# Vi-Sri/CerebralSignalNetworks

Hardware: AMD Instinct MI355X
Metric: EEG-segments/sec training (128ch x 500, hidden=768) (higher is better)
Workload: dtype bf16

## Files before the change

### cerebralsignalnetworks_amd/csrc/csn_common.h

```cpp
#pragma once
#include <hip/hip_runtime.h>
#include <stdint.h>
#include <stdio.h>
#include <stdlib.h>
#include <atomic>
#include <string>

#include "../../include/csn_hip.h"

namespace csn {

typedef __bf16 bf16_t;
typedef __attribute__((ext_vector_type(8))) __bf16 bf16x8;
typedef __attribute__((ext_vector_type(4))) __bf16 bf16x4;
typedef __attribute__((ext_vector_type(4))) float f32x4;
typedef __attribute__((ext_vector_type(4))) short s16x4;

void set_error(const std::string& msg);
int fail(int status, const char* fmt, ...);

#define CSN_HIP_CHECK(expr)                                                              \
  do {                                                                                   \
    hipError_t _e = (expr);                                                              \
    if (_e != hipSuccess)                                                                \
      return ::csn::fail(CSN_ERR_HIP, "%s failed: %s (%s:%d)", #expr, hipGetErrorString(_e), \
                         __FILE__, __LINE__);                                            \
  } while (0)

#define CSN_LAUNCH_CHECK()                                                               \
  do {                                                                                   \
    hipError_t _e = hipGetLastError();                                                   \
    if (_e != hipSuccess)                                                                \
      return ::csn::fail(CSN_ERR_HIP, "kernel launch failed: %s (%s:%d)",                \
                         hipGetErrorString(_e), __FILE__, __LINE__);                     \
  } while (0)

#define CSN_REQUIRE(cond, ...)                                                           \
  do {                                                                                   \
    if (!(cond)) return ::csn::fail(CSN_ERR_INVALID_ARGUMENT, __VA_ARGS__);              \
  } while (0)

struct Options {
  bool cell_v1, no_persist, no_persist_bwd, persist_streams, no_xcd_local, no_rotate, no_fuse_x, no_beside,
      no_side_stream, fwd_ksplit, fwd_nsplit, fwd_flags, bwd_flags, dpoll_no_hint, fwd_hint, gemm_no_dma, gemm_no_256, gemm_generic, tn_no_tr, tn_no_stagger, filter_v1, tags_no_rearm, gemm_no_192, no_half_tiles, nt_no_w4, no_fwd_park;
  int chunk;
  int tn_stages;
};
static inline Options options_from_env() {
  auto on = [](const char* name) { return getenv(name) != nullptr; };
  auto num = [](const char* name, int dflt) {
    const char* e = getenv(name);
    return e ? atoi(e) : dflt;
  };
  Options o{};
  o.cell_v1 = on("CSN_CELL_V1");
  o.no_persist = on("CSN_NO_PERSIST");
  o.no_persist_bwd = on("CSN_NO_PERSIST_BWD");
  o.persist_streams = on("CSN_PERSIST_STREAMS");
  o.no_xcd_local = on("CSN_NO_XCD_LOCAL");
  o.no_rotate = on("CSN_NO_ROTATE");
  o.no_fuse_x = on("CSN_NO_FUSE_X");
  o.no_beside = on("CSN_NO_BESIDE");
  o.no_half_tiles = on("CSN_NO_HALF_TILES");
  o.no_fwd_park = on("CSN_NO_FWD_PARK");
  o.no_side_stream = on("CSN_NO_SIDE_STREAM");
  o.fwd_ksplit = on("CSN_FWD_KSPLIT");
  o.fwd_nsplit = on("CSN_FWD_NSPLIT");
  o.fwd_flags = on("CSN_FWD_FLAGS");
  o.bwd_flags = on("CSN_BWD_FLAGS");
  o.dpoll_no_hint = on("CSN_DPOLL_NO_HINT");
  o.fwd_hint = on("CSN_FWD_HINT");
  o.tn_no_stagger = on("CSN_TN_NO_STAGGER");
  o.gemm_no_dma = on("CSN_GEMM_NO_DMA");
  o.gemm_no_256 = on("CSN_GEMM_NO_256");
  o.gemm_no_192 = on("CSN_GEMM_NO_192");
  o.nt_no_w4 = on("CSN_NT_NO_W4");
  o.gemm_generic = on("CSN_GEMM_GENERIC");
  o.tn_no_tr = on("CSN_TN_NO_TR");
  o.filter_v1 = on("CSN_FILTER_V1");
#ifdef CSN_SLAB_TAGS
  o.tags_no_rearm = on("CSN_TAGS_NO_REARM");
#endif
  o.chunk = num("CSN_LSTM_CHUNK", 32);
  if (o.chunk < 1) o.chunk = 1;
  o.tn_stages = num("CSN_TN_STAGES", 4);
  return o;
}

static inline hipStream_t as_stream(csnStream_t s) { return reinterpret_cast<hipStream_t>(s); }
template <auto Kernel>
static int ensure_dyn_lds(int bytes) {
  static std::atomic<unsigned> done{0u};
  int dev = 0;
  CSN_HIP_CHECK(hipGetDevice(&dev));
  const unsigned bit = 1u << (dev & 31);
  if ((done.load(std::memory_order_acquire) & bit) == 0u) {
    CSN_HIP_CHECK(hipFuncSetAttribute(reinterpret_cast<const void*>(Kernel), hipFuncAttributeMaxDynamicSharedMemorySize, bytes));
    done.fetch_or(bit, std::memory_order_release);
  }
  return CSN_OK;
}

static inline size_t align_up(size_t v, size_t a) { return (v + a - 1) / a * a; }
static inline size_t dtype_size(int dtype) { return dtype == CSN_BF16 ? 2 : 4; }

__device__ __forceinline__ float to_f32(float v) { return v; }
__device__ __forceinline__ float to_f32(bf16_t v) { return (float)v; }
template <typename T> __device__ __forceinline__ T from_f32(float v);
template <> __device__ __forceinline__ float from_f32<float>(float v) { return v; }
template <> __device__ __forceinline__ bf16_t from_f32<bf16_t>(float v) { return (bf16_t)v; }

__device__ __forceinline__ float sigmoid_f32(float x) { return 1.0f / (1.0f + expf(-x)); }
__device__ __forceinline__ float tanh_f32(float x) { return tanhf(x); }

struct CellFwdOne {
// ... 45 lines not shown
```

### cerebralsignalnetworks_amd/csrc/gemm_beside.h

```cpp
#pragma once
#include "gemm_tile.h"
#include "lstm_cell_blk.h"

namespace csn {

static constexpr int kBesideStages = 3;
static constexpr unsigned kBesideStageBytes = 49152;
static constexpr unsigned kBesideLdsBytes = kBesideStages * kBesideStageBytes;

__device__ __forceinline__ void beside_gemm_tiles(const BesideGemm& g, char* smem, unsigned worker, unsigned nworkers) {
  constexpr int NSTAGE = kBesideStages;
  const int tid = threadIdx.x, lane = tid & 63, wave = tid >> 6;
  const int wm = wave >> 1, wn = wave & 1;
  const int64_t M = g.M, N = g.N, K = g.K;
  const unsigned ntn = (unsigned)((N + 127) / 128);
  const unsigned ntiles = ntn * (unsigned)((M + 255) / 256);
  const int nk = (int)(K / 64);
  const unsigned sw = (unsigned)((lane & 15) >> 1);
  const unsigned a_base = (unsigned)((wm * 128 + (lane & 15)) * 128) + ((((unsigned)lane >> 4) ^ sw) << 4);
  const unsigned b_base = 32768u + (unsigned)((wn * 64 + (lane & 15)) * 128) + ((((unsigned)lane >> 4) ^ sw) << 4);

  for (unsigned lid = worker; lid < ntiles; lid += nworkers) {
    __syncthreads();
    const int64_t m0 = (int64_t)(lid / ntn) * 256, n0 = (int64_t)(lid % ntn) * 128;
    const int srow = lane >> 3;
    auto issue = [&](int kt) {
      char* a_s = smem + (kt % NSTAGE) * kBesideStageBytes;
      char* b_s = a_s + 32768;
#pragma unroll
      for (int i = 0; i < 8; ++i) {
        const int row = (4 * i + wave) * 8 + srow;
        const int ch = (lane & 7) ^ ((row >> 1) & 7);
        int64_t am = m0 + row;
        am = am < M ? am : M - 1;
        glds16(g.A + am * K + (int64_t)kt * 64 + ch * 8, a_s + (4 * i + wave) * 1024);
      }
#pragma unroll
      for (int i = 0; i < 4; ++i) {
        const int row = (4 * i + wave) * 8 + srow;
        const int ch = (lane & 7) ^ ((row >> 1) & 7);
        int64_t bn = n0 + row;
        bn = bn < N ? bn : N - 1;
        glds16(g.Bt + bn * K + (int64_t)kt * 64 + ch * 8, b_s + (4 * i + wave) * 1024);
      }
    };

    f32x4 acc[8][4];
#pragma unroll
    for (int i = 0; i < 8; ++i)
#pragma unroll
      for (int j = 0; j < 4; ++j) acc[i][j] = (f32x4){0.f, 0.f, 0.f, 0.f};

#pragma unroll
    for (int h = 0; h < NSTAGE - 1; ++h)
      if (h < nk) issue(h);
    for (int kt = 0; kt < nk; ++kt) {
      const int ahead = nk - 1 - kt;
      if (ahead >= NSTAGE - 2) asm volatile("s_waitcnt vmcnt(%0)" ::"n"(12 * (NSTAGE - 2)) : "memory");
      else asm volatile("s_waitcnt vmcnt(0)" ::: "memory");
      __builtin_amdgcn_s_barrier();
      if (kt + NSTAGE - 1 < nk) issue(kt + NSTAGE - 1);
      const unsigned sb = (unsigned)(kt % NSTAGE) * kBesideStageBytes;
#pragma unroll
      for (int kk = 0; kk < 2; ++kk) {
        const unsigned xo = kk ? 64u : 0u;
        bf16x8 af[8], bfr[4];
#pragma unroll
        for (int j = 0; j < 4; ++j) bfr[j] = lds_read_b128(((b_base ^ xo) + sb) + j * 2048u);
#pragma unroll
        for (int i = 0; i < 8; ++i) af[i] = lds_read_b128(((a_base ^ xo) + sb) + i * 2048u);
#pragma unroll
        for (int i = 0; i < 8; ++i) {
          switch (7 - i) {
            case 7: asm volatile("s_waitcnt lgkmcnt(7)" ::: "memory"); break;
            case 6: asm volatile("s_waitcnt lgkmcnt(6)" ::: "memory"); break;
            case 5: asm volatile("s_waitcnt lgkmcnt(5)" ::: "memory"); break;
            case 4: asm volatile("s_waitcnt lgkmcnt(4)" ::: "memory"); break;
            case 3: asm volatile("s_waitcnt lgkmcnt(3)" ::: "memory"); break;
            case 2: asm volatile("s_waitcnt lgkmcnt(2)" ::: "memory"); break;
            case 1: asm volatile("s_waitcnt lgkmcnt(1)" ::: "memory"); break;
            default: asm volatile("s_waitcnt lgkmcnt(0)" ::: "memory"); break;
          }
          __builtin_amdgcn_sched_barrier(0);
#pragma unroll
          for (int j = 0; j < 4; ++j)
            acc[i][j] = __builtin_amdgcn_mfma_f32_16x16x32_bf16(bfr[j], af[i], acc[i][j], 0, 0, 0);
          __builtin_amdgcn_sched_barrier(0);
        }
      }
    }

#pragma unroll
    for (int i = 0; i < 8; ++i) {
      const int64_t m = m0 + wm * 128 + i * 16 + (lane & 15);
      if (m >= M) continue;
#pragma unroll
      for (int j = 0; j < 4; ++j) {
        const int64_t n = n0 + wn * 64 + j * 16 + (lane >> 4) * 4;
        if (n + 3 < N) {
          *reinterpret_cast<float4*>(g.C + m * N + n) = make_float4(acc[i][j][0], acc[i][j][1], acc[i][j][2], acc[i][j][3]);
        } else {
          for (int r = 0; r < 4; ++r)
            if (n + r < N) g.C[m * N + n + r] = acc[i][j][r];
        }
      }
    }
  }
  asm volatile("s_waitcnt vmcnt(0)" ::: "memory");
}

}
```

### cerebralsignalnetworks_amd/csrc/gemm_nt.hip

```cpp
#include "gemm_tile.h"

namespace csn {

template <typename OutT>
__global__ void __launch_bounds__(256)
gemm_nt_bf16_kernel(const bf16_t* __restrict__ A, const bf16_t* __restrict__ Bt, const float* __restrict__ bias,
                    OutT* __restrict__ C, int64_t M, int64_t N, int64_t K, int accumulate) {
  extern __shared__ __attribute__((aligned(16))) char smem[];
  const int tid = threadIdx.x, lane = tid & 63, wave = tid >> 6;
  const int wm = wave >> 1, wn = wave & 1;
  const unsigned ntn = (unsigned)((N + 127) / 128);
  const unsigned lid = xcd_remap(blockIdx.x, gridDim.x);
  const int64_t m0 = (int64_t)(lid / ntn) * 128, n0 = (int64_t)(lid % ntn) * 128;
  const int nk = (int)((K + 63) / 64);

  uint4 ra[4], rb[4];
  auto load_tile = [&](int kt) {
#pragma unroll
    for (int i = 0; i < 4; ++i) {
      const int q = tid + i * 256;
      const int row = q >> 3, ch = q & 7;
      const int64_t k = (int64_t)kt * 64 + ch * 8;
      const int64_t am = m0 + row, bn = n0 + row;
      ra[i] = (am < M && k < K) ? *reinterpret_cast<const uint4*>(A + am * K + k) : make_uint4(0, 0, 0, 0);
// ... 318 lines not shown
  issue_a(0);
  issue_b(0);
  if (nk > 1) issue_a(1);
  for (int kt = 0; kt < nk; ++kt) {
    if (kt + 1 < nk) asm volatile("s_waitcnt vmcnt(4)" ::: "memory");
    else asm volatile("s_waitcnt vmcnt(0)" ::: "memory");
    __builtin_amdgcn_s_barrier();
    if (kt + 1 < nk) issue_b(kt + 1);
    if (kt + 2 < nk) issue_a(kt + 2);
    const unsigned sa = (unsigned)(kt % 3) * 32768u, sb = (unsigned)(kt % 2) * kBStage;
#pragma unroll
    for (int kk = 0; kk < 2; ++kk) {
      const unsigned xo = kk ? 64u : 0u;
      bf16x8 af[4], bfr[NBF];
#pragma unroll
      for (int j = 0; j < NBF; ++j) bfr[j] = lds_read_b128(((b_base ^ xo) + sb) + j * 2048u);
#pragma unroll
      for (int i = 0; i < 4; ++i) af[i] = lds_read_b128(((a_base ^ xo) + sa) + i * 2048u);
#pragma unroll
      for (int i = 0; i < 4; ++i) {
        if (i == 0) asm volatile("s_waitcnt lgkmcnt(3)" ::: "memory");
        else if (i == 1) asm volatile("s_waitcnt lgkmcnt(2)" ::: "memory");
        else if (i == 2) asm volatile("s_waitcnt lgkmcnt(1)" ::: "memory");
        else asm volatile("s_waitcnt lgkmcnt(0)" ::: "memory");
        __builtin_amdgcn_sched_barrier(0);
#pragma unroll
        for (int j = 0; j < NBF; ++j)
          acc[i][j] = __builtin_amdgcn_mfma_f32_16x16x32_bf16(bfr[j], af[i], acc[i][j], 0, 0, 0);
        __builtin_amdgcn_sched_barrier(0);
      }
    }
  }

#pragma unroll
  for (int i = 0; i < 4; ++i) {
    const int64_t m = m0 + wm * 64 + i * 16 + (lane & 15);
    if (m >= M) continue;
#pragma unroll
    for (int j = 0; j < NBF; ++j) {
      const int64_t n = n0 + wn * (BN / 2) + j * 16 + (lane >> 4) * 4;
      const f32x4 v = nt_with_bias(acc[i][j], bias, n);
#if defined(CSN_NT_ABL) && CSN_NT_ABL == 1
      if (v[0] == v[0]) continue;
#endif
      nt_store4<OutT>(v, C, m * N + n, accumulate);
    }
  }
  }
}

#ifndef CSN_NT_W4_NA
#define CSN_NT_W4_NA 3
#endif
__device__ __forceinline__ int nt64_sw(int row) {
  const int g = (row >> 2) & 3;
  return (((g ^ (g >> 1)) & 1) << 1) | (g >> 1);
}
template <typename OutT, int NA>
__global__ void __launch_bounds__(256, 2)
gemm_nt_w4_kernel(const bf16_t* __restrict__ A, const bf16_t* __restrict__ Bt, const float* __restrict__ bias,
                  OutT* __restrict__ C, int64_t M, int64_t N, int64_t K, int accumulate) {
  static_assert(NA == 2 || NA == 3, "A ring depth");
  constexpr unsigned kAStage = 16384u, kBStage = 12288u, kBBase = NA * kAStage;
  static_assert(kBBase + 2 * kBStage <= 81920u, "two workgroups per CU");
  extern __shared__ __attribute__((aligned(1024))) char smem[];
  const int tid = threadIdx.x, lane = tid & 63;
  const int wave = __builtin_amdgcn_readfirstlane(tid >> 6);
  const int wm = wave >> 1, wn = wave & 1;
  const unsigned ntn = (unsigned)(N / 192);
  const unsigned lid = xcd_remap(blockIdx.x, gridDim.x);
  const int64_t m0 = (int64_t)(lid / ntn) * 256, n0 = (int64_t)(lid % ntn) * 192;
  const int nk = __builtin_amdgcn_readfirstlane((int)(K / 32));

  unsigned a_off[4], b_off[3];
#pragma unroll
  for (int i = 0; i < 4; ++i) {
    const int row = (4 * i + wave) * 16 + (lane >> 2);
    const int ch = (lane & 3) ^ nt64_sw(row);
    int64_t am = m0 + row;
    am = am < M ? am : M - 1;
    a_off[i] = (unsigned)((am * K + ch * 8) * 2);
  }
#pragma unroll
  for (int i = 0; i < 3; ++i) {
    const int row = (4 * i + wave) * 16 + (lane >> 2);
    const int ch = (lane & 3) ^ nt64_sw(row);
    b_off[i] = (unsigned)(((n0 + row) * K + ch * 8) * 2);
  }
  auto issue_a = [&](int kt, int i) {
    glds16(reinterpret_cast<const char*>(A + (int64_t)kt * 32) + a_off[i], smem + (unsigned)(kt % NA) * kAStage + (4 * i + wave) * 1024);
  };
  auto issue_b = [&](int kt, int i) {
    glds16(reinterpret_cast<const char*>(Bt + (int64_t)kt * 32) + b_off[i], smem + kBBase + (unsigned)(kt & 1) * kBStage + (4 * i + wave) * 1024);
  };

  const unsigned frag = (unsigned)((lane & 15) * 64) + ((((unsigned)lane >> 4) ^ (unsigned)nt64_sw(lane & 15)) << 4);
  const unsigned a_base = (unsigned)(wm * 128 * 64) + frag;
  const unsigned b_base = kBBase + (unsigned)(wn * 96 * 64) + frag;
#define W4_READ(addr, off) ({ bf16x8 v_; asm volatile("ds_read_b128 %0, %1 offset:%2" : "=v"(v_) : "v"(addr), "n"(off) : "memory"); v_; })

  f32x4 acc[8][6];
#pragma unroll
  for (int i = 0; i < 8; ++i)
#pragma unroll
    for (int j = 0; j < 6; ++j) acc[i][j] = (f32x4){0.f, 0.f, 0.f, 0.f};

#pragma unroll
  for (int i = 0; i < 4; ++i) issue_a(0, i);
#pragma unroll
  for (int i = 0; i < 3; ++i) issue_b(0, i);
// ... 128 lines not shown
```

### cerebralsignalnetworks_amd/csrc/gemm_tile.h

```cpp
#pragma once
#include "csn_common.h"

namespace csn {

__device__ __forceinline__ unsigned xcd_remap(unsigned bid, unsigned nwg) {
  const unsigned q = nwg >> 3, r = nwg & 7, xcd = bid & 7, slot = bid >> 3;
  return (xcd < r ? xcd * (q + 1) : r * (q + 1) + (xcd - r) * q) + slot;
}

__device__ __forceinline__ int nt_lds_off(int row, int chunk) {
  return row * 128 + ((chunk ^ ((row >> 1) & 7)) << 4);
}

__device__ __forceinline__ int tn_lds_off(int krow, int col) {
  const int s = (krow & 3) | (((krow >> 3) & 1) << 2);
  return krow * 256 + ((((col >> 4) ^ s) << 4) + (col & 15)) * 2;
}
__device__ __forceinline__ int tn256_lds_off(int krow, int col) {
  const int sw = (krow & 3) | (((krow >> 3) & 1) << 2);
  return krow * 512 + ((((col >> 4) ^ sw) << 4) + (col & 15)) * 2;
}

typedef __attribute__((address_space(3))) void* lds_ptr_t;
typedef const __attribute__((address_space(1))) void* gbl_ptr_t;

__device__ __forceinline__ void glds16(const void* g, void* l) {
  __builtin_amdgcn_global_load_lds((gbl_ptr_t)g, (lds_ptr_t)l, 16, 0, 0);
}

template <bool CLAMP>
__device__ __forceinline__ const bf16_t* nt_dma_src(const bf16_t* P, int64_t r0, int64_t rows, int64_t K, int piece, int lane) {
  const int row = piece * 8 + (lane >> 3);
  const int ch = (lane & 7) ^ ((row >> 1) & 7);
  int64_t r = r0 + row;
  if (CLAMP) r = r < rows ? r : rows - 1;
  return P + r * K + ch * 8;
}

__device__ __forceinline__ bf16x8 lds_read_b128(unsigned addr) {
  bf16x8 v;
  asm volatile("ds_read_b128 %0, %1" : "=v"(v) : "v"(addr) : "memory");
  return v;
}

template <typename OutT>
__device__ __forceinline__ void nt_store4(f32x4 v, OutT* __restrict__ C, int64_t idx, int accumulate) {
  if constexpr (sizeof(OutT) == 4) {
    f32x4* dst = reinterpret_cast<f32x4*>((float*)C + idx);
    if (accumulate) v += *dst;
    *dst = v;
  } else {
    *reinterpret_cast<bf16x4*>((bf16_t*)C + idx) = (bf16x4){(bf16_t)v[0], (bf16_t)v[1], (bf16_t)v[2], (bf16_t)v[3]};
  }
}
template <typename OutT>
__device__ __forceinline__ void nt_store1(float v, OutT* __restrict__ C, int64_t idx, int accumulate) {
  if constexpr (sizeof(OutT) == 4) {
    float* dst = (float*)C + idx;
    *dst = accumulate ? *dst + v : v;
  } else {
    ((bf16_t*)C)[idx] = (bf16_t)v;
  }
}
__device__ __forceinline__ f32x4 nt_with_bias(f32x4 v, const float* __restrict__ bias, int64_t n) {
// ... 33 lines not shown
```

### cerebralsignalnetworks_amd/csrc/lstm.hip

```cpp
#include <algorithm>
#include <cstring>
#include <vector>

#include "csn_common.h"
#include "lstm_cell_blk.h"
#include "lstm_cell_common.h"
#include "lstm_dropout.h"
#include "lstm_f32_persist.h"
#include "lstm_resident.h"

namespace csn {

struct LayerWs {
  size_t wih, whh, whht, wiht, whh_blk, whht_blk, bias, xproj, gates, c_all, h_all, dgates, dx, dc_carry, hblk[2],
      dgblk[2], h_blk_all, counters, dg_blk_all, bflags;
  size_t h_drop;
};
struct WsLayout {
  LayerWs layer[8];
  size_t x_c, x_blk, wih0_blk, dy_tm, tn_scratch, colsum, status, agree, agree_b, zeros_bh, f32_bias_part, total;
  size_t zero_fwd, zero_fwd_bytes, zero_bwd, zero_bwd_bytes;
  bool fuse_x;
  bool il, persist, persist_bwd;
  bool fwd_ns;
// ... 1579 lines not shown
      const int cr = r / Cz;
      const bool last = (r == T - 1);
      if (l > 0 || last) {
        if ((rc = hand_off(sc, st, side))) return rc;
      }
      if (l > 0) {
        if ((rc = dx_chunk_gemm(C, l, cr, A.dh_n, side))) return rc;
        hipEvent_t ev;
        if ((rc = next_event(sc, &ev))) return rc;
        CSN_HIP_CHECK(hipEventRecord(ev, side));
        dx_ready[(size_t)l * nch + cr] = ev;
      } else if (last && A.dx != nullptr) {
        if ((rc = dx_out(C, A.dx, side))) return rc;
      }
      if (last && (rc = weight_grads_blk(C, A, l, side))) return rc;
    }
  }
  if ((rc = prof_end(C, 1, n_launch, n_cells))) return rc;
  if ((rc = hand_off(sc, side, st))) return rc;
  for (int l = NL - 1; l >= 0; --l) C.P.grads_ready(l);
  return CSN_OK;
}

static int backward_persist(Call& C, const BwdArgs& A) {
  Plan& P = C.P;
  const WsLayout& w = C.w;
  Prof& g_prof = P.prof;
  char* ws = C.ws;
  hipStream_t st = C.st;
  const float* dh_n = A.dh_n;
  const int B = C.B, T = C.T, H = C.H, NL = C.NL;
  const int64_t G = C.G;
  const int Bpad = (B + 63) / 64 * 64, MT = Bpad / 64;
  const int Cz = C.Cz;
  const int nch = (T + Cz - 1) / Cz;
  const bool beside = NL > 1 && NL <= 4 && bwd_persist_slices(H) <= 28 && G % 64 == 0 && !P.opt.no_beside;
  const int lag = beside ? 2 : 1;
  const int ndiag = nch + lag * (NL - 1);
  int rc;
  CSN_HIP_CHECK(hipMemsetAsync(ws + w.zero_bwd, 0, w.zero_bwd_bytes, st));
  for (int l = 0; l < NL; ++l)
    if ((rc = seed_dc_carry(C, l, A.dc_n, true))) return rc;
  struct DhAdd { int l, t_lo, t_hi; };
  auto add_dh_n = [&](const DhAdd& q) -> int {
    return add_dh_n_rows(C, dh_n + (size_t)(q.l - 1) * B * H, (float*)(ws + w.layer[q.l].dx), q.t_lo, q.t_hi, st);
  };
  const bool try_local = !P.opt.no_xcd_local;

  PersistBwdArgs a{};
  a.error_flag = (unsigned*)(ws + w.status);
  a.B = B; a.H = H; a.T = T; a.Bpad = Bpad; a.MT = MT;
  a.xcd_groups = 1;
  a.grid_slices = 32;
  a.rotate = !P.opt.no_rotate;
  a.data_polls = P.opt.bwd_flags ? 0 : (P.opt.dpoll_no_hint ? 2 : 1);
#ifdef CSN_SLAB_TAGS
  if (a.data_polls && P.opt.tags_no_rearm) a.data_polls |= 4;
#endif
  P.dgates_copies = 2;
  if (a.data_polls)
    for (int l = 0; l < NL; ++l) CSN_HIP_CHECK(hipMemsetAsync(ws + w.layer[l].dg_blk_all, 0xff, (size_t)4 * Bpad * G * 2, st));
  int n_launch = 0;
  P.half_launches[1] = 0;
  BesideGemm pending[3];
  DhAdd pending_add[3] = {{0, 0, 0}, {0, 0, 0}, {0, 0, 0}};
  DhAdd pending_drop[3] = {{0, 0, 0}, {0, 0, 0}, {0, 0, 0}};
  int npending = 0;
  if ((rc = prof_mark(g_prof, 2, st))) return rc;
  for (int dg = 0; dg < ndiag; ++dg) {
    int lay[4], chk[4], ns = 0;
    for (int l = NL - 1; l >= 0; --l) {
      const int c = dg - lag * (NL - 1 - l);
      if (c < 0 || c >= nch) continue;
      const LayerWs& L = w.layer[l];
      PersistBwdSlot& S = a.slot[ns];
      S.wt_blk = (const bf16_t*)(ws + L.whht_blk);
      S.gates = (const bf16_t*)(ws + L.gates);
      S.c_all = (const float*)(ws + L.c_all);
      if (l == NL - 1) {
        S.dy = A.dy_tm;
        S.dy_last = A.dy_tm ? nullptr : A.dy_last;
      } else {
        S.dy = (const float*)(ws + w.layer[l + 1].dx);
        S.dy_last = nullptr;
      }
      S.zeros = (const float*)(ws + w.zeros_bh);
      S.dc_carry = (float*)(ws + L.dc_carry);
      S.dgates = (bf16_t*)(ws + L.dgates);
      S.dg_blk_all = (bf16_t*)(ws + L.dg_blk_all);
      S.flags = (unsigned*)(ws + L.bflags);
      const Chunk k = chunk_at(C, c);
      S.t_hi = T - 1 - k.t0;
      S.nsteps = k.nsteps;
      lay[ns] = l;
      chk[ns] = c;
      ++ns;
    }
    if (ns == 0) {
      for (int i = 0; i < npending; ++i) {
        const BesideGemm& g = pending[i];
        if ((rc = gemm_nt(g.A, g.Bt, nullptr, g.C, g.M, g.N, g.K, CSN_BF16, CSN_F32, 0, st, P.opt))) return rc;
        if ((rc = drop_bwd(C, pending_drop[i].l - 1, pending_drop[i].t_lo, pending_drop[i].t_hi, st))) return rc;
        if (pending_add[i].l && (rc = add_dh_n(pending_add[i]))) return rc;
      }
      npending = 0;
      continue;
// ... 307 lines not shown
```

### cerebralsignalnetworks_amd/csrc/lstm_bwd_persist.hip

```cpp
#include "csn_common.h"
#include "lstm_cell_common.h"
#include "lstm_cell_blk.h"
#include "gemm_beside.h"

#ifdef CSN_PSTAMPS
#ifndef CSN_STAMP_BLOCK
#define CSN_STAMP_BLOCK 11
#endif
__device__ unsigned long long g_bstamps[16];
#define CSN_BSTAMP(i)                                                          \
  do {                                                                         \
    __builtin_amdgcn_sched_barrier(0);                                         \
    if (tid == 0 && blockIdx.x == CSN_STAMP_BLOCK) {                           \
      const unsigned long long now_ = wall_clock64();                          \
      atomicAdd(&g_bstamps[i], now_ - last_);                                  \
      last_ = now_;                                                            \
    }                                                                          \
    __builtin_amdgcn_sched_barrier(0);                                         \
  } while (0)
#else
#define CSN_BSTAMP(i)
#endif

namespace csn {
// ... 4 lines not shown

static constexpr int kBwdRedTile = 68;
__device__ __forceinline__ int bwd_red_pos(int r, int q) { return (r >> 1) + 8 * (r & 1) + 17 * q; }

typedef __attribute__((ext_vector_type(4))) unsigned bu32x4;

__device__ __forceinline__ bf16x8 bload_sc1_b128(__amdgpu_buffer_rsrc_t rsrc, unsigned byte_off, int soff = 0) {
  bu32x4 v = __builtin_amdgcn_raw_buffer_load_b128(rsrc, (int)byte_off, soff, 16);
  union { bu32x4 u; bf16x8 b; } cvt;
  cvt.u = v;
  return cvt.b;
}
template <bool WT>
__device__ __forceinline__ void bstore_b128(__amdgpu_buffer_rsrc_t rsrc, unsigned byte_off, const bf16x8& v, int soff = 0) {
  union { bu32x4 u; bf16x8 b; } cvt;
  cvt.b = v;
  __builtin_amdgcn_raw_buffer_store_b128(cvt.u, rsrc, (int)byte_off, soff, WT ? 16 : 0);
}

struct PersistLens { const int* lengths; };
struct PersistNoLens {};
template <bool MASK> struct PersistLensArg { typedef PersistNoLens type; };
template <> struct PersistLensArg<true> { typedef PersistLens type; };

template <int NUT, int KS, bool DPOLL, bool MASK = false, int RG = 4>
__global__ void __launch_bounds__(256) lstm_bwd_persist_kernel(PersistBwdArgs a, typename PersistLensArg<MASK>::type lens) {
#ifndef CSN_BWD_RING
#define CSN_BWD_RING 5
#endif
  constexpr int RING = KS >= 32 ? 3 : (KS < CSN_BWD_RING ? KS : CSN_BWD_RING);
  static_assert(RG == 4 || RG == 2, "tiles of 64 or 32 rows");
  constexpr int NT = RG * NUT;
  constexpr int QPR = 4 * NUT;
  constexpr int NPAIR = 16 * RG * QPR;
  constexpr int NPASS = NPAIR / 256;
  static_assert(NPAIR % 256 == 0, "tile must split evenly over the 256 threads");
  extern __shared__ __attribute__((aligned(16))) float4 red[];
  const int B = a.B, H = a.H, MT = a.MT, T = a.T;
  const int tid = threadIdx.x, lane = tid & 63, wave = tid >> 6;
#ifdef CSN_PSTAMPS
  const unsigned long long t_entry_ = wall_clock64();
#endif
  const int nslices = H / (16 * NUT);
  int grp, slice;
  if (a.xcd_groups) {
    grp = blockIdx.x & 7;
    slice = blockIdx.x >> 3;
    const int ngroups = a.nslots * MT, gs = a.grid_slices;
    if (grp >= ngroups || slice >= nslices) {
      if (a.ngemm > 0) {
        const int idle_here = gs - nslices;
        const unsigned base = grp <= ngroups ? (unsigned)(grp * idle_here)
                                             : (unsigned)(ngroups * idle_here + (grp - ngroups) * gs);
        const unsigned worker = base + (unsigned)(grp < ngroups ? slice - nslices : slice);
        const unsigned nworkers = (unsigned)(ngroups * idle_here + (8 - ngroups) * gs);
        for (int i = 0; i < a.ngemm; ++i) beside_gemm_tiles(a.gemm[i], reinterpret_cast<char*>(red), worker, nworkers);
      }
      return;
    }
  } else {
    grp = blockIdx.x / nslices;
    slice = blockIdx.x % nslices;
  }
  const PersistBwdSlot& S = a.slot[grp / MT];
  const int mt = grp % MT;
  const int u0 = slice * 16 * NUT, m0 = mt * 16 * RG;
  const int K = 4 * H, kblocks = K >> 5;
  const int ks_beg = wave * KS;
  const size_t slab = (size_t)a.Bpad * K;
  const bf16_t* const wt_blk = S.wt_blk;
  const bf16_t* const gates = S.gates;
  const float* const c_all = S.c_all;
  const float* const dy = S.dy;
  const float* const dy_last = S.dy_last;
  bf16_t* const dgates = S.dgates;
  bf16_t* const dg_blk_all = S.dg_blk_all;
  unsigned* const flags = S.flags + (size_t)mt * kPersistFlagLine;
  const size_t flag_step = (size_t)MT * kPersistFlagLine;
  const int t_hi = S.t_hi, nsteps = S.nsteps;
  constexpr bool dpoll = DPOLL;

  bool local = false;
  if (a.xcd_groups && a.agree != nullptr) {
    if (tid == 0) {
      const unsigned xcc = __builtin_amdgcn_s_getreg(6164) & 7u;
      const unsigned long long mine = 1ull | (1ull << (8 + 6 * xcc));
      __hip_atomic_fetch_add(a.agree + grp, mine, __ATOMIC_RELAXED, __HIP_MEMORY_SCOPE_AGENT);
      const unsigned long long t_begin = wall_clock64();
      unsigned long long v;
      while (((v = __hip_atomic_load(a.agree + grp, __ATOMIC_RELAXED, __HIP_MEMORY_SCOPE_AGENT)) & 0xffull) <
             (unsigned long long)nslices) {
        __builtin_amdgcn_s_sleep(1);
        if (__hip_atomic_load(a.error_flag, __ATOMIC_RELAXED, __HIP_MEMORY_SCOPE_AGENT) != 0u) break;
        if (wall_clock64() - t_begin > kBwdSpinTimeoutTicks) {
          __hip_atomic_store(a.error_flag, 1u, __ATOMIC_RELAXED, __HIP_MEMORY_SCOPE_AGENT);
          break;
        }
      }
      ((__attribute__((address_space(3))) int*)(__attribute__((address_space(3))) void*)red)[0] = (int)(((v >> (8 + 6 * xcc)) & 63ull) == (unsigned long long)nslices);
    }
    __syncthreads();
    local = ((__attribute__((address_space(3))) int*)(__attribute__((address_space(3))) void*)red)[0] != 0;
    __syncthreads();
  }

  const int rot = a.rotate ? (slice * KS) / nslices : 0;
  bf16x8 wreg[KS][NUT];
#pragma unroll
  for (int kb = 0; kb < KS; ++kb) {
// ... 323 lines not shown
        bstore_b128<false>(slabs_rsrc, o1, hi, dst_off);
      } else {
        bstore_b128<true>(slabs_rsrc, o0, lo, dst_off);
        bstore_b128<true>(slabs_rsrc, o1, hi, dst_off);
      }
      bf16x8* op = reinterpret_cast<bf16x8*>(dgates + ((size_t)t * B + row) * K + 4 * (size_t)uq);
      nt_store(op, lo);
      nt_store(op + 1, hi);
      dcn[ps] = make_float4(dcarry[0], dcarry[1], dcarry[2], dcarry[3]);
      cc[ps] = cpv[ps];
    }
    CSN_BSTAMP(3);
    if (!dpoll) asm volatile("s_waitcnt vmcnt(0)" ::: "memory");
    __syncthreads();
    CSN_BSTAMP(4);
    if (!dpoll && tid == 0) {
      unsigned* fl = flags + (size_t)t * flag_step + slice;
      if (local) *fl = 1u;
      else __hip_atomic_store(fl, 1u, __ATOMIC_RELAXED, __HIP_MEMORY_SCOPE_AGENT);
    }
    CSN_BSTAMP(5);
  }

#pragma unroll
  for (int ps = 0; ps < NPASS; ++ps)
    if (pok[ps]) *reinterpret_cast<float4*>(S.dc_carry + (size_t)prow[ps] * H + puq[ps]) = dcn[ps];
}

bool bwd_persist_supported(int B, int H, int dtype, const Options& opt) {
  if (dtype != CSN_BF16 || opt.no_persist || opt.no_persist_bwd) return false;
  return H == 128 || H == 256 || H == 384 || H == 512 || H == 768 || H == 1024;
}
int bwd_persist_slices(int H) { return H / 32; }

template <int NUT, int KS>
static int launch_bwd_persist_t(const PersistBwdArgs& a, hipStream_t st, const int* lengths) {
  size_t lds = (size_t)4 * (a.half_tiles ? 2 : 4) * NUT * kBwdRedTile * sizeof(float4);
  if (lengths != nullptr) {
    if (int rc = ensure_dyn_lds<&lstm_bwd_persist_kernel<NUT, KS, false, true>>((int)kBesideLdsBytes)) return rc;
    if (int rc = ensure_dyn_lds<&lstm_bwd_persist_kernel<NUT, KS, true, true>>((int)kBesideLdsBytes)) return rc;
  } else if (a.half_tiles) {
    if (int rc = ensure_dyn_lds<&lstm_bwd_persist_kernel<NUT, KS, false, false, 2>>((int)kBesideLdsBytes)) return rc;
    if (int rc = ensure_dyn_lds<&lstm_bwd_persist_kernel<NUT, KS, true, false, 2>>((int)kBesideLdsBytes)) return rc;
  } else {
    if (int rc = ensure_dyn_lds<&lstm_bwd_persist_kernel<NUT, KS, false>>((int)kBesideLdsBytes)) return rc;
    if (int rc = ensure_dyn_lds<&lstm_bwd_persist_kernel<NUT, KS, true>>((int)kBesideLdsBytes)) return rc;
  }
  const unsigned nslices = (unsigned)(a.H / (16 * NUT));
  PersistBwdArgs b = a;
  if (b.xcd_groups) {
    if (b.ngemm > 0) {
      lds = kBesideLdsBytes;
      if (b.grid_slices < (int)nslices) b.grid_slices = (int)nslices;
    } else {
      b.grid_slices = (int)nslices;
    }
  }
  const unsigned grid = b.xcd_groups ? 8u * (unsigned)b.grid_slices : nslices * (unsigned)(b.MT * b.nslots);
  if (lengths != nullptr) {
    const PersistLens pl{lengths};
    if (b.data_polls) lstm_bwd_persist_kernel<NUT, KS, true, true><<<dim3(grid), 256, lds, st>>>(b, pl);
    else lstm_bwd_persist_kernel<NUT, KS, false, true><<<dim3(grid), 256, lds, st>>>(b, pl);
  } else if (b.half_tiles) {
    if (b.data_polls) lstm_bwd_persist_kernel<NUT, KS, true, false, 2><<<dim3(grid), 256, lds, st>>>(b, PersistNoLens{});
    else lstm_bwd_persist_kernel<NUT, KS, false, false, 2><<<dim3(grid), 256, lds, st>>>(b, PersistNoLens{});
  } else if (b.data_polls) lstm_bwd_persist_kernel<NUT, KS, true><<<dim3(grid), 256, lds, st>>>(b, PersistNoLens{});
  else lstm_bwd_persist_kernel<NUT, KS, false><<<dim3(grid), 256, lds, st>>>(b, PersistNoLens{});
  CSN_LAUNCH_CHECK();
  return CSN_OK;
}

int launch_bwd_persist(const PersistBwdArgs& a, hipStream_t st, const int* lengths) {
  CSN_REQUIRE(a.nslots >= 1 && a.nslots <= 4 && a.MT >= 1, "launch_bwd_persist: bad slot count");
  const int ns = bwd_persist_slices(a.H);
  CSN_REQUIRE(ns % 4 == 0 && ns <= kPersistFlagLine, "launch_bwd_persist: H=%d gives %d slices", a.H, ns);
  if (a.xcd_groups) CSN_REQUIRE(a.nslots * a.MT <= 8, "launch_bwd_persist: groups do not fit 8 XCDs");
  CSN_REQUIRE(a.MT * (a.half_tiles ? 32 : 64) == a.Bpad, "launch_bwd_persist: %d tiles of %d rows are not Bpad=%d", a.MT,
              a.half_tiles ? 32 : 64, a.Bpad);
  CSN_REQUIRE(!a.half_tiles || (a.xcd_groups && lengths == nullptr), "launch_bwd_persist: 32-row groups need the grouped form and no lengths");
  CSN_REQUIRE(a.ngemm >= 0 && a.ngemm <= 3 && (a.ngemm == 0 || a.xcd_groups), "launch_bwd_persist: bad GEMM list");
  for (int i = 0; i < a.ngemm; ++i)
    CSN_REQUIRE(a.gemm[i].K % 64 == 0 && a.gemm[i].N % 4 == 0 && a.gemm[i].M > 0, "launch_bwd_persist: GEMM %d shape", i);
  switch (a.H) {
    case 1024: return launch_bwd_persist_t<2, 32>(a, st, lengths);
    case 768: return launch_bwd_persist_t<2, 24>(a, st, lengths);
    case 512: return launch_bwd_persist_t<2, 16>(a, st, lengths);
    case 384: return launch_bwd_persist_t<2, 12>(a, st, lengths);
    case 256: return launch_bwd_persist_t<2, 8>(a, st, lengths);
    case 128: return launch_bwd_persist_t<2, 4>(a, st, lengths);
  }
  return fail(CSN_ERR_UNSUPPORTED, "launch_bwd_persist: no kernel for H=%d", a.H);
}

}

#ifdef CSN_PSTAMPS
extern "C" int csn_debug_read_bstamps(unsigned long long* out) {
  unsigned long long z[16] = {0};
  if (hipMemcpyFromSymbol(out, HIP_SYMBOL(g_bstamps), sizeof(z)) != hipSuccess) return 1;
  if (hipMemcpyToSymbol(HIP_SYMBOL(g_bstamps), z, sizeof(z)) != hipSuccess) return 1;
  return 0;
}
#endif
```

### cerebralsignalnetworks_amd/csrc/lstm_cell_blk.h

```cpp
#pragma once
#include "csn_common.h"

#ifdef CSN_SLAB_TAGS
#define CSN_DPOLL_MODE(x) ((x) & 3)
#define CSN_DPOLL_NO_REARM(x) (((x) & 4) != 0)
#else
#define CSN_DPOLL_MODE(x) (x)
#define CSN_DPOLL_NO_REARM(x) false
#endif

namespace csn {

struct CellFwdProb {
  const bf16_t* h_prev_blk;
  const bf16_t* w_blk;
  const float* xproj;
  const float* c_prev;
  bf16_t* gates_out;
  float* c_out;
  bf16_t* h_out;
  bf16_t* h_out_blk;
};
struct CellFwdArgs {
  CellFwdProb p[4];
// ... 31 lines not shown
  int I;
  int t0, nsteps;
};
struct BesideGemm {
  const bf16_t* A;
  const bf16_t* Bt;
  float* C;
  int M, N, K;
};
static constexpr int kPersistFlagLine = 32;
struct PersistFwdArgs {
  PersistFwdSlot slot[4];
  int nslots;
  int data_polls;
  int xcd_groups;
  int rotate;
  unsigned long long* agree;
  unsigned* error_flag;
  int B, H, T, Bpad, MT;
  int state;
  int half_tiles;
  int park;
};
static constexpr int kRedTile = 71;
static constexpr int kParkSlots = 6;
constexpr size_t fwd_persist_lds_bytes(int nq, bool park) {
  return (size_t)(4 * 4 * nq * kRedTile + 4 * nq + (park ? kParkSlots * 256 : 0)) * 16;
}
bool fwd_persist_supported(int B, int H, int dtype, const Options& opt);
bool fwd_ns_supported(int B, int H, int dtype, const Options& opt);
int fwd_ns_slices(int H);
int launch_fwd_ns(const PersistFwdArgs& a, hipStream_t st);
int fwd_persist_slices(int H);
int launch_fwd_persist(const PersistFwdArgs& a, hipStream_t st);

struct PersistBwdSlot {
  const bf16_t* wt_blk;
  const bf16_t* gates;
  const float* c_all;
  const float* dy;
  const float* dy_last;
  const float* zeros;
  float* dc_carry;
  bf16_t* dgates;
  bf16_t* dg_blk_all;
  unsigned* flags;
  int t_hi, nsteps;
};
struct PersistBwdArgs {
  PersistBwdSlot slot[4];
  int nslots;
  BesideGemm gemm[3];
  int ngemm;
  int grid_slices;
  int xcd_groups;
  int rotate;
  int data_polls;
  unsigned long long* agree;
  unsigned* error_flag;
  int B, H, T, Bpad, MT;
  int half_tiles;
};
bool bwd_persist_supported(int B, int H, int dtype, const Options& opt);
int bwd_persist_slices(int H);
int launch_bwd_persist(const PersistBwdArgs& a, hipStream_t st, const int* lengths = nullptr);

enum { kPrepBlockify = 0, kPrepPermRows, kPrepTransPerm, kPrepBias, kPrepCastX, kPrepBlockifyX };
static constexpr int kPrepMaxJobs = 32;
struct PrepJob {
  int kind;
  const float* a;
  const float* b;
  void* dst;
  int64_t n0, n1, n2, s0, s1, H;
  int perm_r, perm_k;
  int64_t work;
  unsigned blk_begin, blk_count;
  const int* len;
};
struct PrepArgs {
  PrepJob job[kPrepMaxJobs];
  int njobs;
  const int* vrow;
  const int* vt0;
};
static_assert(sizeof(PrepArgs) <= 4096, "PrepArgs is passed by value: the kernel-argument segment holds 4096 bytes");
int launch_prep_multi(PrepArgs& A, hipStream_t st);

bool cell_blk_supported(int H, int dtype, const Options& opt);
int launch_cell_fwd_il(const CellFwdArgs& a, int nprob, hipStream_t st);
int launch_cell_bwd_il(const CellBwdArgs& a, int nprob, hipStream_t st, const CellMask* mask = nullptr);
int launch_blockify_x(const float* x, int64_t xsb, int64_t xst, int B, int T, int I, void* dst, hipStream_t st);
int launch_blockify(const float* src, int64_t ld_r, int64_t ld_k, int64_t R, int64_t K, int perm_r, int perm_k,
                    int64_t H, void* dst, hipStream_t st);
int launch_permute_rows_cast(const float* src, int64_t H, int64_t I, void* dst, hipStream_t st);
int launch_transpose_perm_cast(const float* src, int64_t H, int64_t I, void* dst, hipStream_t st);
int launch_bias_perm_sum(const float* a, const float* b, int64_t H, float* dst, hipStream_t st);
int launch_reduce_slabs_unperm(const float* slabs, int64_t slab_stride, int S, int64_t H, int64_t C, float* out,
                               float* out2, int accumulate, hipStream_t st);

}
```

Baseline: 27790.

## Add wide 256x192 beside-GEMM tile path with XCD-local tile walk

Adds a second beside-GEMM path for the persistent backward kernel. It uses 256x192 tiles with a 4-stage LDS ring, direct global-to-LDS loads interleaved with MFMA, and a tile walk that keeps contiguous panels on each XCD. A host heuristic picks the wide path per GEMM when N is divisible by 192 and it needs noticeably fewer rounds than the 128-wide tiles; an env flag forces the old path. The goal is higher reuse per tile and fewer rounds for the weight-gradient GEMMs that run beside the recurrence, at the cost of a larger accumulator register footprint and hand-tuned waitcnt scheduling.

```diff
diff --git a/cerebralsignalnetworks_amd/csrc/csn_common.h b/cerebralsignalnetworks_amd/csrc/csn_common.h
--- a/cerebralsignalnetworks_amd/csrc/csn_common.h
+++ b/cerebralsignalnetworks_amd/csrc/csn_common.h
@@ -41,7 +41,7 @@
   } while (0)
 
 struct Options {
-  bool cell_v1, no_persist, no_persist_bwd, persist_streams, no_xcd_local, no_rotate, no_fuse_x, no_beside,
+  bool cell_v1, no_persist, no_persist_bwd, persist_streams, no_xcd_local, no_rotate, no_fuse_x, no_beside, beside_128,
       no_side_stream, fwd_ksplit, fwd_nsplit, fwd_flags, bwd_flags, dpoll_no_hint, fwd_hint, gemm_no_dma, gemm_no_256, gemm_generic, tn_no_tr, tn_no_stagger, filter_v1, tags_no_rearm, gemm_no_192, no_half_tiles, nt_no_w4, no_fwd_park;
   int chunk;
   int tn_stages;
@@ -61,6 +61,7 @@
   o.no_rotate = on("CSN_NO_ROTATE");
   o.no_fuse_x = on("CSN_NO_FUSE_X");
   o.no_beside = on("CSN_NO_BESIDE");
+  o.beside_128 = on("CSN_BESIDE_128");
   o.no_half_tiles = on("CSN_NO_HALF_TILES");
   o.no_fwd_park = on("CSN_NO_FWD_PARK");
   o.no_side_stream = on("CSN_NO_SIDE_STREAM");
diff --git a/cerebralsignalnetworks_amd/csrc/gemm_beside.h b/cerebralsignalnetworks_amd/csrc/gemm_beside.h
--- a/cerebralsignalnetworks_amd/csrc/gemm_beside.h
+++ b/cerebralsignalnetworks_amd/csrc/gemm_beside.h
@@ -8,7 +8,123 @@
 static constexpr unsigned kBesideStageBytes = 49152;
 static constexpr unsigned kBesideLdsBytes = kBesideStages * kBesideStageBytes;
 
-__device__ __forceinline__ void beside_gemm_tiles(const BesideGemm& g, char* smem, unsigned worker, unsigned nworkers) {
+#ifndef CSN_BESIDE_WIDE_STAGES
+#define CSN_BESIDE_WIDE_STAGES 4
+#endif
+static constexpr int kBesideWideStages = CSN_BESIDE_WIDE_STAGES;
+static constexpr unsigned kBesideWideStageBytes = 16384 + 12288;
+static_assert(kBesideWideStages >= 3 && kBesideWideStages * kBesideWideStageBytes <= kBesideLdsBytes, "wide ring depth");
+
+struct BesideWalk { unsigned first, end, step; };
+__host__ __device__ __forceinline__ BesideWalk beside_xcd_tiles(unsigned npanels, unsigned ntn, unsigned xbase, unsigned xcount,
+                                                                unsigned local, unsigned nworkers) {
+  const unsigned p0 = npanels * xbase / nworkers, p1 = npanels * (xbase + xcount) / nworkers;
+  return BesideWalk{p0 * ntn + local, p1 * ntn, xcount};
+}
+
+#define CSN_BESIDE_VMCNT(n) asm volatile("s_waitcnt vmcnt(%0)" ::"n"(n) : "memory")
+
+__device__ __forceinline__ void beside_gemm_tiles_wide(const BesideGemm& g, char* smem, const BesideWalk walk) {
+  constexpr int NS = kBesideWideStages;
+  constexpr unsigned kStage = kBesideWideStageBytes, kBOff = 16384u;
+  const int tid = threadIdx.x, lane = tid & 63;
+  const int wave = __builtin_amdgcn_readfirstlane(tid >> 6);
+  const int wm = wave >> 1, wn = wave & 1;
+  const int64_t M = g.M, N = g.N, K = g.K;
+  const unsigned ntn = (unsigned)(N / 192);
+  const int nk = __builtin_amdgcn_readfirstlane((int)(K / 32));
+  const unsigned frag = (unsigned)((lane & 15) * 64) + ((((unsigned)lane >> 4) ^ (unsigned)nt64_sw(lane & 15)) << 4);
+  const unsigned a_base = (unsigned)(wm * 128 * 64) + frag;
+  const unsigned b_base = kBOff + (unsigned)(wn * 96 * 64) + frag;
+#define BESIDE_READ(addr, off) ({ bf16x8 v_; asm volatile("ds_read_b128 %0, %1 offset:%2" : "=v"(v_) : "v"(addr), "n"(off) : "memory"); v_; })
+
+  for (unsigned lid = walk.first; lid < walk.end; lid += walk.step) {
+    __syncthreads();
+    const int64_t m0 = (int64_t)(lid / ntn) * 256, n0 = (int64_t)(lid % ntn) * 192;
+    const char* const a_tile = reinterpret_cast<const char*>(g.A + m0 * K);
+    const char* const b_tile = reinterpret_cast<const char*>(g.Bt + n0 * K);
+    const int last = (int)(M - m0 < 256 ? M - m0 : 256) - 1;
+    unsigned a_off[4], b_off[3];
+#pragma unroll
+    for (int i = 0; i < 4; ++i) {
+      const int row = (4 * i + wave) * 16 + (lane >> 2);
+      const int ch = (lane & 3) ^ nt64_sw(row);
+      a_off[i] = (unsigned)(((int64_t)(row < last ? row : last) * K + ch * 8) * 2);
+    }
+#pragma unroll
+    for (int i = 0; i < 3; ++i) {
+      const int row = (4 * i + wave) * 16 + (lane >> 2);
+      const int ch = (lane & 3) ^ nt64_sw(row);
+      b_off[i] = (unsigned)(((int64_t)row * K + ch * 8) * 2);
+    }
+    auto issue = [&](int kt, unsigned slot, int p) {
+      char* const s = smem + slot * kStage;
+      if (p < 4) glds16(a_tile + (int64_t)kt * 64 + a_off[p], s + (4 * p + wave) * 1024);
+      else glds16(b_tile + (int64_t)kt * 64 + b_off[p - 4], s + kBOff + (4 * (p - 4) + wave) * 1024);
+    };
+
+    f32x4 acc[8][6];
+#pragma unroll
+    for (int i = 0; i < 8; ++i)
+#pragma unroll
+      for (int j = 0; j < 6; ++j) acc[i][j] = (f32x4){0.f, 0.f, 0.f, 0.f};
+
+#pragma unroll
+    for (int h = 0; h < NS - 1; ++h)
+      if (h < nk) {
+#pragma unroll
+        for (int p = 0; p < 7; ++p) issue(h, (unsigned)h, p);
+      }
+    unsigned cur = 0, nxt = NS - 1;
+    for (int kt = 0; kt < nk; ++kt) {
+      const int ahead = nk - 1 - kt;
+      if (ahead >= NS - 2) CSN_BESIDE_VMCNT(7 * (NS - 2));
+      else if (NS > 4 && ahead == 2) CSN_BESIDE_VMCNT(14);
+      else if (NS > 3 && ahead == 1) CSN_BESIDE_VMCNT(7);
+      else CSN_BESIDE_VMCNT(0);
+      __builtin_amdgcn_s_barrier();
+      const bool more = kt + NS - 1 < nk;
+      const unsigned aa = a_base + cur * kStage, ba = b_base + cur * kStage;
+      bf16x8 af[2], bfr[6];
+#pragma unroll
+      for (int j = 0; j < 6; ++j) bfr[j] = BESIDE_READ(ba, j * 1024);
+      af[0] = BESIDE_READ(aa, 0);
+#pragma unroll
+      for (int i = 0; i < 8; ++i) {
+        if (i < 7) af[(i + 1) & 1] = BESIDE_READ(aa, (i + 1) * 1024);
+        if (i < 7) asm volatile("s_waitcnt lgkmcnt(1)" ::: "memory");
+        else asm volatile("s_waitcnt lgkmcnt(0)" ::: "memory");
+        __builtin_amdgcn_sched_barrier(0);
+#pragma unroll
+        for (int j = 0; j < 6; ++j) {
+          acc[i][j] = __builtin_amdgcn_mfma_f32_16x16x32_bf16(bfr[j], af[i & 1], acc[i][j], 0, 0, 0);
+          __builtin_amdgcn_sched_barrier(0);
+          if (j == 1 && i < 7) {
+            if (more) issue(kt + NS - 1, nxt, i);
+            __builtin_amdgcn_sched_barrier(0);
+          }
+        }
+      }
+      cur = cur + 1 == NS ? 0 : cur + 1;
+      nxt = nxt + 1 == NS ? 0 : nxt + 1;
+    }
+
+#pragma unroll
+    for (int i = 0; i < 8; ++i) {
+      const int64_t m = m0 + wm * 128 + i * 16 + (lane & 15);
+      if (m >= M) continue;
+#pragma unroll
+      for (int j = 0; j < 6; ++j) {
+        const int64_t n = n0 + wn * 96 + j * 16 + (lane >> 4) * 4;
+        *reinterpret_cast<float4*>(g.C + m * N + n) = make_float4(acc[i][j][0], acc[i][j][1], acc[i][j][2], acc[i][j][3]);
+      }
+    }
+  }
+#undef BESIDE_READ
+  asm volatile("s_waitcnt vmcnt(0)" ::: "memory");
+}
+
+__device__ __forceinline__ void beside_gemm_tiles_narrow(const BesideGemm& g, char* smem, unsigned worker, unsigned nworkers) {
   constexpr int NSTAGE = kBesideStages;
   const int tid = threadIdx.x, lane = tid & 63, wave = tid >> 6;
   const int wm = wave >> 1, wn = wave & 1;
@@ -108,5 +224,37 @@
   }
   asm volatile("s_waitcnt vmcnt(0)" ::: "memory");
 }
-
-}
+#undef CSN_BESIDE_VMCNT
+
+static inline bool beside_takes_wide(int64_t M, int64_t N, int ngroups, int nslices, int grid_slices) {
+  if (N % 192 != 0) return false;
+  const unsigned idle = (unsigned)(grid_slices - nslices), nworkers = (unsigned)ngroups * idle + (unsigned)(8 - ngroups) * grid_slices;
+  if (nworkers == 0) return false;
+  const unsigned npanels = (unsigned)((M + 255) / 256), ntn = (unsigned)(N / 192);
+  unsigned wide_rounds = 0, base = 0;
+  for (int x = 0; x < 8; ++x) {
+    const unsigned count = x < ngroups ? idle : (unsigned)grid_slices;
+    if (count == 0) continue;
+    const BesideWalk w = beside_xcd_tiles(npanels, ntn, base, count, 0, nworkers);
+    const unsigned rounds = (w.end - w.first + count - 1) / count;
+    wide_rounds = rounds > wide_rounds ? rounds : wide_rounds;
+    base += count;
+  }
+  const unsigned narrow_rounds = (npanels * (unsigned)((N + 127) / 128) + nworkers - 1) / nworkers;
+  return wide_rounds < 2 || 13 * wide_rounds <= 10 * narrow_rounds;
+}
+
+__device__ __forceinline__ void beside_gemm_tiles(const BesideGemm& g, char* smem, unsigned xbase, unsigned xcount, unsigned local,
+                                                  unsigned nworkers, bool wide) {
+  if (wide) {
+    const unsigned npanels = (unsigned)((g.M + 255) / 256), ntn = (unsigned)(g.N / 192);
+#ifdef CSN_BESIDE_WIDE_RR
+    beside_gemm_tiles_wide(g, smem, BesideWalk{xbase + local, npanels * ntn, nworkers});
+#else
+    beside_gemm_tiles_wide(g, smem, beside_xcd_tiles(npanels, ntn, xbase, xcount, local, nworkers));
+#endif
+  } else
+    beside_gemm_tiles_narrow(g, smem, xbase + local, nworkers);
+}
+
+}
diff --git a/cerebralsignalnetworks_amd/csrc/gemm_nt.hip b/cerebralsignalnetworks_amd/csrc/gemm_nt.hip
--- a/cerebralsignalnetworks_amd/csrc/gemm_nt.hip
+++ b/cerebralsignalnetworks_amd/csrc/gemm_nt.hip
@@ -394,10 +394,6 @@
 #ifndef CSN_NT_W4_NA
 #define CSN_NT_W4_NA 3
 #endif
-__device__ __forceinline__ int nt64_sw(int row) {
-  const int g = (row >> 2) & 3;
-  return (((g ^ (g >> 1)) & 1) << 1) | (g >> 1);
-}
 template <typename OutT, int NA>
 __global__ void __launch_bounds__(256, 2)
 gemm_nt_w4_kernel(const bf16_t* __restrict__ A, const bf16_t* __restrict__ Bt, const float* __restrict__ bias,
diff --git a/cerebralsignalnetworks_amd/csrc/gemm_tile.h b/cerebralsignalnetworks_amd/csrc/gemm_tile.h
--- a/cerebralsignalnetworks_amd/csrc/gemm_tile.h
+++ b/cerebralsignalnetworks_amd/csrc/gemm_tile.h
@@ -10,6 +10,11 @@
 
 __device__ __forceinline__ int nt_lds_off(int row, int chunk) {
   return row * 128 + ((chunk ^ ((row >> 1) & 7)) << 4);
+}
+
+__device__ __forceinline__ int nt64_sw(int row) {
+  const int g = (row >> 2) & 3;
+  return (((g ^ (g >> 1)) & 1) << 1) | (g >> 1);
 }
 
 __device__ __forceinline__ int tn_lds_off(int krow, int col) {
diff --git a/cerebralsignalnetworks_amd/csrc/lstm.hip b/cerebralsignalnetworks_amd/csrc/lstm.hip
--- a/cerebralsignalnetworks_amd/csrc/lstm.hip
+++ b/cerebralsignalnetworks_amd/csrc/lstm.hip
@@ -1655,6 +1655,7 @@
   a.B = B; a.H = H; a.T = T; a.Bpad = Bpad; a.MT = MT;
   a.xcd_groups = 1;
   a.grid_slices = 32;
+  a.beside_narrow = P.opt.beside_128 ? 1 : 0;
   a.rotate = !P.opt.no_rotate;
   a.data_polls = P.opt.bwd_flags ? 0 : (P.opt.dpoll_no_hint ? 2 : 1);
 #ifdef CSN_SLAB_TAGS
diff --git a/cerebralsignalnetworks_amd/csrc/lstm_bwd_persist.hip b/cerebralsignalnetworks_amd/csrc/lstm_bwd_persist.hip
--- a/cerebralsignalnetworks_amd/csrc/lstm_bwd_persist.hip
+++ b/cerebralsignalnetworks_amd/csrc/lstm_bwd_persist.hip
@@ -80,9 +80,11 @@
         const int idle_here = gs - nslices;
         const unsigned base = grp <= ngroups ? (unsigned)(grp * idle_here)
                                              : (unsigned)(ngroups * idle_here + (grp - ngroups) * gs);
-        const unsigned worker = base + (unsigned)(grp < ngroups ? slice - nslices : slice);
+        const unsigned here = (unsigned)(grp < ngroups ? idle_here : gs);
+        const unsigned local = (unsigned)(grp < ngroups ? slice - nslices : slice);
         const unsigned nworkers = (unsigned)(ngroups * idle_here + (8 - ngroups) * gs);
-        for (int i = 0; i < a.ngemm; ++i) beside_gemm_tiles(a.gemm[i], reinterpret_cast<char*>(red), worker, nworkers);
+        for (int i = 0; i < a.ngemm; ++i)
+          beside_gemm_tiles(a.gemm[i], reinterpret_cast<char*>(red), base, here, local, nworkers, ((a.gemm_wide >> i) & 1) != 0);
       }
       return;
     }
@@ -512,6 +514,10 @@
     if (b.ngemm > 0) {
       lds = kBesideLdsBytes;
       if (b.grid_slices < (int)nslices) b.grid_slices = (int)nslices;
+      b.gemm_wide = 0;
+      for (int i = 0; i < b.ngemm; ++i)
+        if (!b.beside_narrow && beside_takes_wide(b.gemm[i].M, b.gemm[i].N, b.nslots * b.MT, (int)nslices, b.grid_slices))
+          b.gemm_wide |= 1 << i;
     } else {
       b.grid_slices = (int)nslices;
     }
@@ -540,7 +546,7 @@
   CSN_REQUIRE(!a.half_tiles || (a.xcd_groups && lengths == nullptr), "launch_bwd_persist: 32-row groups need the grouped form and no lengths");
   CSN_REQUIRE(a.ngemm >= 0 && a.ngemm <= 3 && (a.ngemm == 0 || a.xcd_groups), "launch_bwd_persist: bad GEMM list");
   for (int i = 0; i < a.ngemm; ++i)
-    CSN_REQUIRE(a.gemm[i].K % 64 == 0 && a.gemm[i].N % 4 == 0 && a.gemm[i].M > 0, "launch_bwd_persist: GEMM %d shape", i);
+    CSN_REQUIRE(a.gemm[i].K % 64 == 0 && a.gemm[i].K <= (1 << 22) && a.gemm[i].N % 4 == 0 && a.gemm[i].M > 0, "launch_bwd_persist: GEMM %d shape", i);
   switch (a.H) {
     case 1024: return launch_bwd_persist_t<2, 32>(a, st, lengths);
     case 768: return launch_bwd_persist_t<2, 24>(a, st, lengths);
diff --git a/cerebralsignalnetworks_amd/csrc/lstm_cell_blk.h b/cerebralsignalnetworks_amd/csrc/lstm_cell_blk.h
--- a/cerebralsignalnetworks_amd/csrc/lstm_cell_blk.h
+++ b/cerebralsignalnetworks_amd/csrc/lstm_cell_blk.h
@@ -107,6 +107,8 @@
   int nslots;
   BesideGemm gemm[3];
   int ngemm;
+  int beside_narrow;
+  int gemm_wide;
   int grid_slices;
   int xcd_groups;
   int rotate;
```

Result: faster. 28190, median of 6 (+1.4%).
